# Emilianogith/MPC-for-dynamic-locomotion-in-the-MIT-cheetah-3

Hardware: AMD Instinct MI355X
Metric: QP solves/sec (horizon=10, 4-contact Lite3) at batch=4096 (higher is better)
Workload: dtype f32 tiles + f64 residuals

## Files before the change

mpc-for-dynamic-locomotion-in-the-mit-cheetah-3_amd/csrc/mpcqp_kernels.hip:

```cpp

#include "mpcqp_wrench.h"
#include "mpcqp_stage.h"
#include "mpcqp_elementwise.h"
#include "mpcqp_model.h"
#include "mpcqp_joints.h"

#include <cstdio>
#include <cstdlib>
#include <cstring>
#include <new>
#include <type_traits>

#ifndef MPCQP_DIAG_LDSPAD
#define MPCQP_DIAG_LDSPAD 0
#endif

struct mpcqp_engine {
  MpcQpConfig cfg;
  DevCfg dev;
  DevCfg* dcfg = nullptr;
  hipEvent_t ev0 = nullptr, ev1 = nullptr;
  int* order_mem = nullptr;
  int order_phase = 0;
  int order_cap = 0;
// ... 276 lines not shown
}

static bool invert_small(int n, const double* A, double* Ai) {
  double* M = new (std::nothrow) double[2 * n * n];
  if (!M) return false;
  for (int i = 0; i < n; ++i)
    for (int j = 0; j < n; ++j) { M[i * 2 * n + j] = A[i * n + j]; M[i * 2 * n + n + j] = i == j ? 1.0 : 0.0; }
  bool ok = true;
  for (int k = 0; k < n && ok; ++k) {
    int piv = k;
    for (int i = k + 1; i < n; ++i) if (fabs(M[i * 2 * n + k]) > fabs(M[piv * 2 * n + k])) piv = i;
    if (!(fabs(M[piv * 2 * n + k]) > 0)) { ok = false; break; }
    if (piv != k) for (int j = 0; j < 2 * n; ++j) { const double t = M[k * 2 * n + j]; M[k * 2 * n + j] = M[piv * 2 * n + j]; M[piv * 2 * n + j] = t; }
    const double p = 1.0 / M[k * 2 * n + k];
    for (int j = 0; j < 2 * n; ++j) M[k * 2 * n + j] *= p;
    for (int i = 0; i < n; ++i) {
      if (i == k) continue;
      const double f = M[i * 2 * n + k];
      if (f != 0) for (int j = 0; j < 2 * n; ++j) M[i * 2 * n + j] -= f * M[k * 2 * n + j];
    }
  }
  if (ok) for (int i = 0; i < n; ++i) for (int j = 0; j < n; ++j) Ai[i * n + j] = M[i * 2 * n + n + j];
  delete[] M;
  return ok;
}

template <int N>
static void lane_order_kinv(const double* Ki, double* lane) {
  constexpr int G = WG<N>::G, NQ = WG<N>::NQ;
  auto S0 = [&](int R, int C) -> double {
    if (R >= NQ || C >= NQ) return R == C ? 1.0 : 0.0;
    return R % 6 == C % 6 ? Ki[((R % 6) * N + R / 6) * N + C / 6] : 0.0;
  };
  for (int t = 0; t < G * G; ++t) {
    const int gr = t / G, gc = t % G, k = ((gr - gc) % 3 + 3) % 3;
    for (int r = 0; r < 8; ++r) {
      const int c0 = (r + 2 * k) % 6;
      lane[16 * t + r] = S0(8 * gr + r, 8 * gc + c0);
      lane[16 * t + 8 + r] = c0 < 2 ? S0(8 * gr + r, 8 * gc + c0 + 6) : 0.0;
    }
  }
}

template <int N>
static int build_wrench_tables(mpcqp_engine* e) {
  const MpcQpConfig& c = e->cfg;
  double* tab = new (std::nothrow) double[2 * N * N];
  double* K = new (std::nothrow) double[6 * N * N];
  double* Ki = new (std::nothrow) double[6 * N * N];
  float* Ki32 = new (std::nothrow) float[6 * N * N];
  constexpr int NLANE = 16 * WG<N>::NT;
  double* Kl = new (std::nothrow) double[NLANE];
  float* Kl32 = new (std::nothrow) float[NLANE];
  int rc = tab && K && Ki && Ki32 && Kl && Kl32 ? MPCQP_OK : MPCQP_ENOMEM;
  if (rc == MPCQP_OK) {
    const double dl = c.delta, th = e->dev.theta;
    for (int a = 0; a < N; ++a)
      for (int bq = 0; bq < N; ++bq) {
        const int mx = a > bq ? a : bq;
        tab[a * N + bq] = dl * dl * (double)(N - mx);
        double sacc = 0;
        for (int k = mx + 1; k <= N; ++k) sacc += ((double)(k - 1 - a) + th) * ((double)(k - 1 - bq) + th);
        tab[N * N + a * N + bq] = dl * dl * dl * dl * sacc;
      }
  }
  for (int q = 0; q < 6 && rc == MPCQP_OK; ++q) {
    for (int i = 0; i < N * N; ++i) K[q * N * N + i] = 2.0 * (c.w[q] * tab[N * N + i] + c.w[6 + q] * tab[i]);
    if (!invert_small(N, K + q * N * N, Ki + q * N * N)) rc = MPCQP_EINVAL;
  }
  if (rc == MPCQP_OK) {
    for (int i = 0; i < 6 * N * N; ++i) Ki32[i] = (float)Ki[i];
    lane_order_kinv<N>(Ki, Kl);
    for (int i = 0; i < NLANE; ++i) Kl32[i] = (float)Kl[i];
    hipError_t he = hipMalloc((void**)&e->wr_K, sizeof(double) * 6 * N * N);
    if (he == hipSuccess) he = hipMemcpy(e->wr_K, K, sizeof(double) * 6 * N * N, hipMemcpyHostToDevice);
    if (he == hipSuccess) he = hipMalloc((void**)&e->wr_kinv32, sizeof(float) * 6 * N * N);
    if (he == hipSuccess) he = hipMemcpy(e->wr_kinv32, Ki32, sizeof(float) * 6 * N * N, hipMemcpyHostToDevice);
    if (he == hipSuccess) he = hipMalloc((void**)&e->wr_kinv64, sizeof(double) * 6 * N * N);
    if (he == hipSuccess) he = hipMemcpy(e->wr_kinv64, Ki, sizeof(double) * 6 * N * N, hipMemcpyHostToDevice);
    if (he == hipSuccess) he = hipMalloc((void**)&e->wr_klane32, sizeof(float) * NLANE);
    if (he == hipSuccess) he = hipMemcpy(e->wr_klane32, Kl32, sizeof(float) * NLANE, hipMemcpyHostToDevice);
    if (he == hipSuccess) he = hipMalloc((void**)&e->wr_klane64, sizeof(double) * NLANE);
    if (he == hipSuccess) he = hipMemcpy(e->wr_klane64, Kl, sizeof(double) * NLANE, hipMemcpyHostToDevice);
    if (he != hipSuccess) { (void)hipGetLastError(); rc = MPCQP_ENOMEM; }
  }
  delete[] tab; delete[] K; delete[] Ki; delete[] Ki32; delete[] Kl; delete[] Kl32;
  return rc;
}

static void free_engine(mpcqp_engine* h) {
  if (h->dcfg) (void)hipFree(h->dcfg);
  if (h->order_mem) (void)hipFree(h->order_mem);
  if (h->dual_mem) (void)hipFree(h->dual_mem);
  if (h->model_mem) (void)hipFree(h->model_mem);
  if (h->gait_mem) (void)hipFree(h->gait_mem);
  if (h->roll_mem) (void)hipFree(h->roll_mem);
  if (h->plan_ws) (void)hipFree(h->plan_ws);
  if (h->wr_K) (void)hipFree(h->wr_K);
  if (h->wr_kinv32) (void)hipFree(h->wr_kinv32);
  if (h->wr_kinv64) (void)hipFree(h->wr_kinv64);
  if (h->wr_klane32) (void)hipFree(h->wr_klane32);
  if (h->wr_klane64) (void)hipFree(h->wr_klane64);
  if (h->stage_ws) (void)hipFree(h->stage_ws);
  if (h->ev0) (void)hipEventDestroy(h->ev0);
  if (h->ev1) (void)hipEventDestroy(h->ev1);
  delete h;
}

extern "C" {

uint32_t mpcqp_version(void) { return MPCQP_VERSION; }

int mpcqp_default_config(MpcQpConfig* c) {
  if (!c) return MPCQP_EINVAL;
  memset(c, 0, sizeof(*c));
  c->size = (uint32_t)sizeof(*c);
  c->N = 10;
  c->delta = 0.03;
  c->m = 8.885;
  c->Ibody_inv[0] = 1.0 / 0.24; c->Ibody_inv[1] = 1.0; c->Ibody_inv[2] = 1.0;
  const double w[13] = {1e4, 2.7e4, 1e4, 2.7e5, 2.7e5, 2.7e5, 1e4, 1e4, 1e4, 1.6e4, 1.6e4, 1.6e4, 0.0};
  memcpy(c->w, w, sizeof(w));
  c->alpha = 1e-2;
  c->f_min = 3.0; c->f_max = 100.0;
  c->disc = MPCQP_DISC_EULER;
  c->dtype = MPCQP_DTYPE_F32;
  c->precision = MPCQP_PREC_MIXED;
  c->flags = MPCQP_FLAG_POLISH;
  c->rho = 1.0; c->sigma = 1e-6; c->relax = 1.6;
  c->max_iter = 400; c->check_every = 100;
  c->eps_abs = 1e-5; c->eps_rel = 1e-6;
  c->polish_max = 4;
  c->device = 0;
  return MPCQP_OK;
}

int mpcqp_create(const MpcQpConfig* cfg, mpcqp_handle* out) {
  if (!cfg || !out || cfg->size != sizeof(MpcQpConfig)) return MPCQP_EINVAL;
  *out = nullptr;
// ... 623 lines not shown
```

mpc-for-dynamic-locomotion-in-the-mit-cheetah-3_amd/csrc/mpcqp_leg.h:

```cpp
#pragma once
#include "mpcqp_common.h"
#include "mpcqp_legmap.h"

namespace {

__device__ __forceinline__ int opaque(int v) { asm volatile("" : "+v"(v)); return v; }
__device__ __forceinline__ double opaque_zero_f64() {
  unsigned lo, hi;
  asm volatile("v_mov_b32 %0, 0\n\tv_mov_b32 %1, 0" : "=v"(lo), "=v"(hi));
  return __builtin_bit_cast(double, ((unsigned long long)hi << 32) | lo);
}
template <typename T> __device__ __forceinline__ T opaque_zero() {
  if constexpr (sizeof(T) == 8) return (T)opaque_zero_f64();
  else { float z; asm volatile("v_mov_b32 %0, 0" : "=v"(z)); return (T)z; }
}
__device__ __forceinline__ float ufloat(float v) { return __builtin_bit_cast(float, __builtin_amdgcn_readfirstlane(__builtin_bit_cast(int, v))); }

template <int NW>
__device__ __forceinline__ void wsync() {
  if constexpr (NW == 1) {
    __builtin_amdgcn_fence(__ATOMIC_RELEASE, "wavefront");
    __builtin_amdgcn_wave_barrier();
    __builtin_amdgcn_fence(__ATOMIC_ACQUIRE, "wavefront");
  } else {
    __syncthreads();
  }
}

template <int Q, int NW>
__device__ __forceinline__ void wmax(float (&v)[Q], float* red, int tid) {
  if constexpr (NW == 1) {
#pragma unroll
    for (int q = 0; q < Q; ++q) v[q] = wave_max(v[q]);
  } else {
    block_max<Q, NW>(v, red, tid);
  }
}

template <int Q, int NW>
__device__ __forceinline__ void wsum(float (&v)[Q], float* red, int tid) {
  if constexpr (NW == 1) {
#pragma unroll
    for (int q = 0; q < Q; ++q) v[q] = wave_sum(v[q]);
  } else {
    block_sum<Q, NW>(v, red, tid);
  }
}

template <typename T> __device__ __forceinline__ T quad_sum(T v) { v += dpp_mov<0xB1>(v); v += dpp_mov<0x4E>(v); return v; }

template <typename T>
__device__ __forceinline__ T rs8(const T (&v)[8], int gc) {
  const bool hi = (gc & 4) != 0, b1 = (gc & 2) != 0, b0 = (gc & 1) != 0;
  T t[4];
#pragma unroll
  for (int m = 0; m < 4; ++m) { const T keep = hi ? v[4 + m] : v[m], send = hi ? v[m] : v[4 + m]; t[m] = keep + dpp_mov<0x141>(send); }
  T s2[2];
#pragma unroll
  for (int m = 0; m < 2; ++m) { const T keep = b1 ? t[2 + m] : t[m], send = b1 ? t[m] : t[2 + m]; s2[m] = keep + dpp_mov<0x4E>(send); }
  const T keep = b0 ? s2[1] : s2[0], send = b0 ? s2[0] : s2[1];
  return keep + dpp_mov<0xB1>(send);
}

__device__ __forceinline__ float w_rcp(float x) { return __builtin_amdgcn_rcpf(x); }
__device__ __forceinline__ double w_rcp(double x) {
  double r = __builtin_amdgcn_rcp(x);
  r = fma(fma(-x, r, 1.0), r, r);
  r = fma(fma(-x, r, 1.0), r, r);
  return r;
}

template <typename TM> __device__ __forceinline__ void ld8(const TM* p, TM (&o)[8]);
template <> __device__ __forceinline__ void ld8<float>(const float* p, float (&o)[8]) {
  const float4 a = reinterpret_cast<const float4*>(p)[0], b = reinterpret_cast<const float4*>(p)[1];
  o[0] = a.x; o[1] = a.y; o[2] = a.z; o[3] = a.w; o[4] = b.x; o[5] = b.y; o[6] = b.z; o[7] = b.w;
}
template <> __device__ __forceinline__ void ld8<double>(const double* p, double (&o)[8]) {
#pragma unroll
  for (int h = 0; h < 4; ++h) { const double2 a = reinterpret_cast<const double2*>(p)[h]; o[2 * h] = a.x; o[2 * h + 1] = a.y; }
}
template <typename TM> __device__ __forceinline__ void st8(TM* p, const TM (&o)[8]);
template <> __device__ __forceinline__ void st8<float>(float* p, const float (&o)[8]) {
  reinterpret_cast<float4*>(p)[0] = make_float4(o[0], o[1], o[2], o[3]);
  reinterpret_cast<float4*>(p)[1] = make_float4(o[4], o[5], o[6], o[7]);
}
template <> __device__ __forceinline__ void st8<double>(double* p, const double (&o)[8]) {
#pragma unroll
  for (int h = 0; h < 4; ++h) reinterpret_cast<double2*>(p)[h] = make_double2(o[2 * h], o[2 * h + 1]);
}


template <typename TM>
struct LegAdmm {
  TM u[3], z[5], yh[5], g[3];
  TM lo0, hi0, loA, hiB;
  TM mu;
};

struct ActSet {
  int zs, xs, ys;
  bool ez, ex, ey;
  __device__ __forceinline__ ActSet(int code, bool stance) {
    zs = (code & 3) - 1; xs = ((code >> 2) & 3) - 1; ys = ((code >> 4) & 3) - 1;
    ez = stance && zs == 0; ex = stance && xs == 0; ey = stance && ys == 0;
  }
};

#ifndef MPCQP_AA_M
#define MPCQP_AA_M 3
#endif
constexpr int AA_M = MPCQP_AA_M;
constexpr int AA_NS = 2 * AA_M;
constexpr int AA_NC = AA_M * (AA_M - 1) / 2;
// ... 172 lines not shown
```

mpc-for-dynamic-locomotion-in-the-mit-cheetah-3_amd/csrc/mpcqp_wrench.h:

```cpp
#pragma once
#include "mpcqp_leg.h"

namespace {

template <int N_>
struct WG {
  static constexpr int N = N_, NL = 4 * N, n = 12 * N, NQ = 6 * N;
  static constexpr int G = N <= 10 ? 8 : 16;
  static constexpr int NT = G * G, NW = NT / 64;
  static constexpr int DP = 8 * G;
  static constexpr int NB = (NQ + 7) / 8;
  static_assert(NQ <= DP, "horizon too long for the lane grid");
};

struct WrTabs {
  const double* K;
  const float* kinv32;
  const double* kinv64;
  const float* klane32;
  const double* klane64;
};

template <typename TV, int N>
struct SmemW {
  using Geo = WG<N>;
  TV x0[13];
  TV mu, cy, sy;
  TV rzw0[3];
  TV wP[6], wQ[6];
  TV delta, theta, alpha, inv_m, fmin, fmax;
  TV alpha_target, alpha_ok;
  TV Bl[Geo::NL * 9];
  TV cm[Geo::NL];
  TV gam[Geo::NQ];
  TV gl[Geo::n];
  TV uv[Geo::n];
  TV ww[Geo::NQ], kap[Geo::NQ];
  union {
    struct { TV pu[Geo::n], py[Geo::NL * 5]; };
    struct { TV rr[Geo::n]; TV xd[(N + 1) * 13]; };
  };
  union {
    struct { TV ua[Geo::n], za[Geo::NL * 5], ya[Geo::NL * 5]; };
    struct { TV e0P[Geo::NQ], e0Q[Geo::NQ]; };
  };
  alignas(16) double E[N * 36];
  alignas(16) double piv[2 * Geo::DP];
  alignas(16) double bv[Geo::DP], cv[Geo::DP];
  float red[Geo::NW * 4];
  float aared[Geo::NW * 12];
  float aah[N > 10 ? 45 * Geo::NL : 1];
  float kkt[4];
  float resid[4];
// ... 94 lines not shown

__device__ __forceinline__ void ld4(const float* p, float (&o)[4]) {
  const f2 a = reinterpret_cast<const f2*>(p)[0], b = reinterpret_cast<const f2*>(p)[1];
  o[0] = a.x; o[1] = a.y; o[2] = b.x; o[3] = b.y;
}
__device__ __forceinline__ void ld4(const double* p, double (&o)[4]) {
  const double2 a = reinterpret_cast<const double2*>(p)[0], b = reinterpret_cast<const double2*>(p)[1];
  o[0] = a.x; o[1] = a.y; o[2] = b.x; o[3] = b.y;
}

__device__ __forceinline__ float wmasked(float x, int m) { return __builtin_bit_cast(float, __builtin_bit_cast(int, x) & m); }
__device__ __forceinline__ double wmasked(double x, int m) { return __builtin_bit_cast(double, __builtin_bit_cast(long long, x) & (long long)m); }

template <typename TM, int N, bool VM>
__device__ __forceinline__ void w_tile_init(WTile<TM>& t, const WKq<TM>& kq, const TM* __restrict__ E, int gr, int gc) {
  constexpr int NQ = WG<N>::NQ, G = WG<N>::G;
  asm volatile("" : "+v"(gr), "+v"(gc));
  const unsigned cls = (unsigned)(gr - gc + 3 * G) % 3u;
  const bool kc[3] = {cls == 0u, cls == 1u, cls == 2u};
#pragma unroll
  for (int r = 0; r < 8; ++r) {
    TM kv[8];
#pragma unroll
    for (int c = 0; c < 8; ++c) {
      TM v = (TM)0;
#pragma unroll
      for (int k = 0; k < 3; ++k) {
        const int c0 = (r + 2 * k) % 6;
        if (c == c0) v = kc[k] ? kq.v0[r] : v;
        else if (c == c0 + 6) v = kc[k] ? kq.v1[r] : v;
      }
      kv[c] = v;
    }
    const int R = 8 * gr + r, jR = (R * 43) >> 8;
    const int h = R < NQ ? 3 * jR - 4 * gc : 64;
    const int base = 6 * R - 2 * h;
    const unsigned bits = ((7u << min((unsigned)(h + 2), 31u)) >> 2) & 15u;
#pragma unroll
    for (int hq = 0; hq < 2; ++hq) {
      const bool in0 = (unsigned)(2 * hq - h) < 3u, in1 = (unsigned)(2 * hq + 1 - h) < 3u;
      TM e[4];
      if constexpr (VM) ld4(E + ((bits & (3u << (2 * hq))) ? base + 4 * hq : 0), e);
      else ld4(E + ((in0 || in1) ? base + 4 * hq : 0), e);
#pragma unroll
      for (int i = 0; i < 4; ++i) {
        const int c = 4 * hq + i;
        if constexpr (VM) tset(t, r, c, kv[c] + wmasked(e[i], __builtin_amdgcn_sbfe((int)bits, 2 * hq + (i >> 1), 1)));
        else tset(t, r, c, kv[c] + ((i < 2 ? in0 : in1) ? e[i] : (TM)0));
      }
    }
  }
}

template <typename TM, int N>
__device__ __forceinline__ void w_sweep(WTile<TM>& t, TM* __restrict__ piv, int gr, int gc) {
  constexpr int NW = WG<N>::NW, DP = WG<N>::DP, G = WG<N>::G;
  int step = 0;
  for (int og = 0; og < G; ++og) {
#pragma unroll
    for (int rr = 0; rr < 8; ++rr) {
      if (8 * og + rr >= WG<N>::NQ) break;
      TM* vb = piv + (NW > 1 ? (step & 1) * DP : 0);
      if (gr == og) {
        TM row[8];
#pragma unroll
        for (int j = 0; j < 8; ++j) row[j] = tget(t, rr, j);
        st8<TM>(vb + 8 * gc, row);
      }
      wsync<NW>();
      const TM p = w_rcp(vb[8 * og + rr]);
      TM vc[8], vr[8];
      ld8<TM>(vb + 8 * gc, vc);
      ld8<TM>(vb + 8 * gr, vr);
      const bool prow = gr == og, pcol = gc == og;
      TM m[8];
#pragma unroll
      for (int i = 0; i < 8; ++i) { vr[i] *= p; m[i] = vr[i]; }
      m[rr] = prow ? (TM)1 - p : vr[rr];
      rank1(t, m, vc);
#pragma unroll
      for (int i = 0; i < 8; ++i) {
        const TM v = (i == rr && prow) ? -p : vr[i];
        tset(t, i, rr, pcol ? v : tget(t, i, rr));
      }
      if constexpr (NW == 1) wsync<1>();
      tpin(t);
      ++step;
    }
  }
}

template <typename TM, int N, bool NEGATE = true>
__device__ __forceinline__ void w_matvec(const WTile<TM>& t, const TM* __restrict__ bv, TM* __restrict__ cv, int gr, int gc) {
  constexpr int G = WG<N>::G;
  TM x[8], acc[8];
  ld8<TM>(bv + 8 * gc, x);
  tilemv(t, x, acc);
  if constexpr (G == 16) {
#pragma unroll
    for (int i = 0; i < 8; ++i) acc[i] += dpp_mov<0x140>(acc[i]);
  }
  const TM sum = rs8<TM>(acc, gc & 7), tot = NEGATE ? -sum : sum;
  if (gc < 8) cv[8 * gr + gc] = tot;
}

template <int N, bool MIXED> constexpr bool W_LEGMAP = N == 10 && MIXED;
template <int N, bool MIXED> constexpr bool W_MED3 = N == 10 && MIXED;

template <typename TM, int N, typename LS>
__device__ __forceinline__ void w_build_E(const LS& L, TM* __restrict__ E, int tid) {
  constexpr int NL = WG<N>::NL, NW = WG<N>::NW;
  TM e[21];
  int k = 0;
  if constexpr (LS::dense) {
#pragma unroll
    for (int q = 0; q < 6; ++q) {
#pragma unroll
      for (int p = q; p < 6; ++p) {
        TM a = L.dinv[0] * L.A[0][q] * L.A[0][p];
        a = fma(L.dinv[1] * L.A[1][q], L.A[1][p], a);
        a = fma(L.dinv[2] * L.A[2][q], L.A[2][p], a);
        e[k++] = quad_sum(a);
      }
    }
  } else {
    L.gram(e, [](TM a) { return quad_sum(a); });
  }
  if (tid < NL && (tid & 3) == 0) {
    TM* Ej = E + 36 * (tid >> 2);
    k = 0;
#pragma unroll
    for (int q = 0; q < 6; ++q) {
#pragma unroll
      for (int p = q; p < 6; ++p) { Ej[6 * q + p] = e[k]; Ej[6 * p + q] = e[k]; ++k; }
    }
  }
  wsync<NW>();
}

template <typename TM, int N, bool QUAD_PIN = false, typename LS>
__device__ __forceinline__ void w_solve(const WTile<TM>& t, const LS& L, const TM (&rhs)[3], TM (&x)[3], TM* __restrict__ bv,
                                        TM* __restrict__ cv, int tid, int gr, int gc) {
  constexpr int NL = WG<N>::NL, NW = WG<N>::NW;
  TM a[3];
#pragma unroll
  for (int c = 0; c < 3; ++c) a[c] = L.dinv[c] * rhs[c];
  TM b[6];
  static_assert(!QUAD_PIN || (sizeof(TM) == 4 && !LS::dense), "the pinned form is written for fp32 on the structured maps");
  if constexpr (LS::dense) {
#pragma unroll
    for (int q = 0; q < 6; ++q) b[q] = quad_sum(fma(L.A[2][q], a[2], fma(L.A[1][q], a[1], L.A[0][q] * a[0])));
  } else if constexpr (!QUAD_PIN) {
    L.wrench(a, b, [](TM v) { return quad_sum(v); });
  } else {
    L.wrench(a, b, [](TM v) { return v; });
    typedef float v2f __attribute__((ext_vector_type(2)));
    v2f p01 = {b[0], b[1]}, p34 = {b[3], b[4]};
    asm volatile("" : "+v"(p01), "+v"(p34));
    b[0] = p01.x; b[1] = p01.y; b[3] = p34.x; b[4] = p34.y;
    asm volatile("" : "+v"(b[2]), "+v"(b[5]));
#pragma unroll
    for (int q = 0; q < 6; ++q) b[q] = quad_sum(b[q]);
  }
  {
    const int l = min(tid & 3, 2);
    TM v0 = l == 0 ? b[0] : (l == 1 ? b[2] : b[4]), v1 = l == 0 ? b[1] : (l == 1 ? b[3] : b[5]);
    if constexpr (QUAD_PIN) { asm volatile("" : "+v"(v0)); asm volatile("" : "+v"(v1)); }
    if (tid < NL) { TM* d = bv + 6 * (tid >> 2) + 2 * l; d[0] = v0; d[1] = v1; }
  }
  wsync<NW>();
  w_matvec<TM, N, !QUAD_PIN>(t, bv, cv, gr, gc);
  wsync<NW>();
  const TM* cj = cv + 6 * (min(tid, NL - 1) >> 2);
  TM c6[6];
#pragma unroll
  for (int q = 0; q < 6; ++q) c6[q] = QUAD_PIN ? -cj[q] : cj[q];
  if constexpr (LS::dense) {
#pragma unroll
    for (int c = 0; c < 3; ++c) {
      TM s = L.A[c][0] * c6[0];
#pragma unroll
      for (int q = 1; q < 6; ++q) s = fma(L.A[c][q], c6[q], s);
      x[c] = a[c] - L.dinv[c] * s;
    }
  } else {
    L.back(c6, [&](const int c, const TM sc) { x[c] = a[c] - L.dinv[c] * sc; });
  }
}

template <typename TV, typename TIO, int N>
__device__ __forceinline__ int w_load(SmemW<TV, N>& s, const FastIn<TIO>& in, size_t b, int tid) {
  constexpr int NT = WG<N>::NT, n = WG<N>::n, NL = WG<N>::NL, NX = (N + 1) * 13;
  constexpr int RX = (NX + NT - 1) / NT, RR = (n + NT - 1) / NT, RC = (NL + NT - 1) / NT;
  TIO vx[RX], vr[RR], v0 = 0, vm = 0;
  uint8_t vc[RC];
  const TIO* xp = in.xdes + b * (size_t)NX;
  const TIO* rp = in.r + b * (size_t)n;
  const uint8_t* cp = in.contact + b * (size_t)NL;
#pragma unroll
  for (int q = 0; q < RX; ++q) { const int i = tid + q * NT; vx[q] = i < NX ? xp[i] : (TIO)0; }
#pragma unroll
  for (int q = 0; q < RR; ++q) { const int i = tid + q * NT; vr[q] = i < n ? rp[i] : (TIO)0; }
#pragma unroll
  for (int q = 0; q < RC; ++q) { const int i = tid + q * NT; vc[q] = i < NL ? cp[i] : (uint8_t)0; }
  if (tid < 13) v0 = in.x0[b * 13 + tid];
  if (tid == 0) vm = in.mu[b];
  int bad = 0;
#pragma unroll
  for (int q = 0; q < RX; ++q) { const int i = tid + q * NT; if (i < NX) { s.xd[i] = (TV)vx[q]; bad |= !isfinite(vx[q]); } }
#pragma unroll
  for (int q = 0; q < RR; ++q) { const int i = tid + q * NT; if (i < n) { s.rr[i] = (TV)vr[q]; bad |= !isfinite(vr[q]); } }
#pragma unroll
  for (int q = 0; q < RC; ++q) { const int i = tid + q * NT; if (i < NL) s.ct[i] = vc[q] ? 1 : 0; }
  if (tid < 13) { s.x0[tid] = (TV)v0; bad |= !isfinite(v0); }
  if (tid == 0) { s.mu = (TV)vm; bad |= !isfinite(vm); }
  return bad;
}

template <typename TV, int N>
__device__ __forceinline__ void w_grad(SmemW<TV, N>& s, const double* __restrict__ Ktab, int tid, TV (&gr)[3]) {
  constexpr int NL = WG<N>::NL, NQ = WG<N>::NQ, NW = WG<N>::NW, NT = WG<N>::NT;
  static_assert(NQ <= NT, "one wrench component per lane");
  const int L = min(tid, NL - 1);
  const int e = min(tid, NQ - 1), ej = e / 6, eq = e - 6 * ej;
// ... 271 lines not shown
  TV u[3], z[5], y[5], g[3];
#pragma unroll
  for (int a = 0; a < 3; ++a) { u[a] = s.ua[3 * L + a]; g[a] = s.gl[3 * L + a]; }
#pragma unroll
  for (int i = 0; i < 5; ++i) { z[i] = s.za[5 * L + i]; y[i] = s.ya[5 * L + i]; }
  return w_ratio<TV, N>(s, tabs, u, z, y, g, s.mu, tid < NL, tid);
}

constexpr double ALPHA_FLOOR = 3e-6;
constexpr int POLISH_CHEAP_LEGS = 3;
constexpr int POLISH_CHEAP_STEPS = 3;
constexpr int POLISH_PATIENCE = 1;

template <typename TV, typename TM, int N, typename LS>
__device__ __forceinline__ void w_admm_sys(const SmemW<TV, N>& s, const DevCfg& cfg, int L, float rho, LS& Ls) {
  const bool stance = s.ct[L] != 0;
  if constexpr (LS::dense) {
#pragma unroll
    for (int c = 0; c < 3; ++c) {
#pragma unroll
      for (int i = 0; i < 3; ++i) Ls.A[c][i] = (TM)s.Bl[9 * L + 3 * i + c];
#pragma unroll
      for (int a = 0; a < 3; ++a) Ls.A[c][3 + a] = a == c ? (TM)s.cm[L] : (TM)0;
    }
  } else {
#pragma unroll
    for (int c = 0; c < 3; ++c) {
#pragma unroll
      for (int i = 0; i < 3; ++i) Ls.B[c][i] = (TM)s.Bl[9 * L + 3 * i + c];
    }
    Ls.cm = (TM)s.cm[L];
  }
  TM sigma = (TM)cfg.sigma;
  if constexpr (sizeof(TM) == 4) sigma = ufloat(sigma);
  const TM r = (TM)rho, m = (TM)s.mu, a2 = (TM)((TV)2 * s.alpha);
  if constexpr (!LS::dense) {
    const TM base = a2 + sigma;
    Ls.dinv[0] = Ls.dinv[1] = stance ? (TM)1 / (base + (r + r)) : (TM)0;
    Ls.dinv[2] = stance ? (TM)1 / fma(r, fma((TM)4 * m, m, (TM)1), base) : (TM)0;
  } else {
    Ls.dinv[0] = Ls.dinv[1] = stance ? (TM)1 / (a2 + sigma + (TM)2 * r) : (TM)0;
    Ls.dinv[2] = stance ? (TM)1 / (a2 + sigma + r * fma((TM)4 * m, m, (TM)1)) : (TM)0;
  }
}

template <typename TV, typename TM, int N, bool REFINE = false>
__device__ __forceinline__ void w_admm(SmemW<TV, N>& s, const DevCfg& cfg, const WrTabs& tabs, const int adapt,
                                       const int kfirst, const int tid0) {
  constexpr int NL = WG<N>::NL, NW = WG<N>::NW, G = WG<N>::G;
  constexpr bool AA_CARRY = NW == 1 && !REFINE && sizeof(TM) == 4;
  constexpr bool LM = W_LEGMAP<N, sizeof(TM) == 4>;
  static_assert(!LM || (NW == 1 && sizeof(TM) == 4), "w_solve's pinned quad sums are written for one wave and fp32");
  constexpr bool MED3 = W_MED3<N, sizeof(TM) == 4>;
  using TS = std::conditional_t<(N > 10), double, TM>;
  TM* const E = reinterpret_cast<TM*>(s.E);
  TM* const piv = reinterpret_cast<TM*>(s.piv);
  TM* const bv = reinterpret_cast<TM*>(s.bv);
  TM* const cv = reinterpret_cast<TM*>(s.cv);
  float rho = s.rho;
  int K = kfirst > 0 ? min(kfirst, cfg.check_every) : cfg.check_every;
  K = max(1, min(K, cfg.max_iter - __builtin_amdgcn_readfirstlane(s.iters)));
  const int seg_len = (!REFINE && sizeof(TM) == 4 && cfg.accel_p > 0 && cfg.accel_restart > 0) ? cfg.accel_restart : (1 << 30);
  const bool check = adapt && cfg.early_check;
  int it = 0, seg_end = min(K, (adapt && ADAPT_AT < K) ? ADAPT_AT : seg_len);
  int hard = 0;
  float ratio = 0.f;
  STAMP_INIT
  for (;;) {
    WKq<TS> kq;
    {
      const int tid = fresh_tid<NW>(tid0), L = min(tid, NL - 1);
      w_kq_load<TS>(kq, w_klane<TS>(tabs), tid);
      typename LegMapPick<LM, LegMapAdmm<TS>, TS>::type Ls;
      w_admm_sys<TV, TS, N>(s, cfg, L, rho, Ls);
      w_build_E<TS, N>(Ls, reinterpret_cast<TS*>(s.E), tid);
    }
    STAMP(1);
    WTile<TM> tile;
    {
      const int tid = fresh_tid<NW>(tid0), gr = tid / G, gc = tid % G;
      if constexpr (sizeof(TS) == sizeof(TM)) {
        w_tile_init<TM, N, sizeof(TM) == 4>(tile, kq, E, gr, gc);
        STAMP(2);
        w_sweep<TM, N>(tile, piv, gr, gc);
      } else {
        WTile<TS> t64;
        w_tile_init<TS, N, sizeof(TM) == 4>(t64, kq, reinterpret_cast<const TS*>(s.E), gr, gc);
        STAMP(2);
        w_sweep<TS, N>(t64, reinterpret_cast<TS*>(s.piv), gr, gc);
#pragma unroll
        for (int i = 0; i < 8; ++i) {
#pragma unroll
          for (int j = 0; j < 4; ++j) tile.v[i][j] = mk2((float)t64.v[i][2 * j], (float)t64.v[i][2 * j + 1]);
        }
      }
    }
    STAMP(3);
    {
      const int tid = fresh_tid<NW>(tid0), L = min(tid, NL - 1), gr = tid / G, gc = tid % G;
      const bool leg = tid < NL, stance = s.ct[L] != 0;
      const TM sigma = (TM)cfg.sigma, relax = (TM)cfg.relax, om = (TM)1 - relax, BIG = (TM)1e30, r = (TM)rho;
      if (tid >= WG<N>::NQ && tid < WG<N>::DP) bv[tid] = (TM)0;
      typename LegMapPick<LM, LegMapAdmm<TM>, TM>::type Ls;
      w_admm_sys<TV, TM, N>(s, cfg, L, rho, Ls);
      LegAdmm<TM> A;
      A.mu = (TM)s.mu;
#pragma unroll
      for (int a = 0; a < 3; ++a) { A.u[a] = (TM)s.ua[3 * L + a]; A.g[a] = (TM)s.gl[3 * L + a]; }
#pragma unroll
      for (int i = 0; i < 5; ++i) { A.z[i] = (TM)s.za[5 * L + i]; A.yh[i] = (TM)(s.ya[5 * L + i] / (TV)rho); }
      A.lo0 = stance ? (TM)s.fmin : (TM)0; A.hi0 = stance ? (TM)s.fmax : (TM)0;
      A.loA = stance ? -BIG : (TM)0; A.hiB = stance ? BIG : (TM)0;
      bool rebuild = false;
      constexpr bool AA_ON = !REFINE && sizeof(TM) == 4, AA_LDS = N > 10;
      const int aa_p = AA_ON ? __builtin_amdgcn_readfirstlane(cfg.accel_p) : 0;
      LegAA aa;
      TM aa_xb[5], aa_fp[5];
      auto aa_park = [&]() {
        if constexpr (AA_LDS) {
          if (leg) {
            float* h = s.aah + L;
#pragma unroll
            for (int k = 0; k < 5; ++k) {
              h[NL * k] = (float)aa_xb[k]; h[NL * (5 + k)] = (float)aa_fp[k]; h[NL * (10 + k)] = aa.rp[k];
#pragma unroll
              for (int j = 0; j < AA_M; ++j) { h[NL * (15 + 5 * j + k)] = aa.dX[j][k]; h[NL * (15 + 5 * AA_M + 5 * j + k)] = aa.dF[j][k]; }
            }
          }
        }
      };
      auto aa_fetch = [&]() {
        if constexpr (AA_LDS) {
          const float* h = s.aah + L;
#pragma unroll
          for (int k = 0; k < 5; ++k) {
            aa_xb[k] = (TM)h[NL * k]; aa_fp[k] = (TM)h[NL * (5 + k)]; aa.rp[k] = h[NL * (10 + k)];
#pragma unroll
// ... 141 lines not shown
    if (y0 + (u2 - fmaxv) > 0) zs = 1;
    else if (y0 + (u2 - fminv) < 0) zs = -1;
    const bool hx = y1 + g1 > 0, lx = y2 + g2 < 0;
    if (hx && lx) xs = (g1 > -g2) ? 1 : -1; else if (hx) xs = 1; else if (lx) xs = -1;
    const bool hy = y3 + g3_ > 0, ly = y4 + g4 < 0;
    if (hy && ly) ys = (g3_ > -g4) ? 1 : -1; else if (hy) ys = 1; else if (ly) ys = -1;
  }
  return (zs + 1) | ((xs + 1) << 2) | ((ys + 1) << 4);
}

template <typename TV, int N>
__device__ __forceinline__ unsigned w_aset_hash(SmemW<TV, N>& s, const int tid) {
  constexpr int NL = WG<N>::NL, NW = WG<N>::NW;
  if (tid == 0) s.ahash = 0u;
  wsync<NW>();
  if (tid < NL) atomicAdd(&s.ahash, ((unsigned)s.aset[tid] + 1u) * (2654435761u * (unsigned)(2 * tid + 1)));
  wsync<NW>();
  const unsigned h = (unsigned)__builtin_amdgcn_readfirstlane((int)s.ahash);
  wsync<NW>();
  return h;
}

#ifndef MPCQP_W_INCR_LEGS
#define MPCQP_W_INCR_LEGS 8
#endif
#ifndef MPCQP_W_INCR_STEPS
#define MPCQP_W_INCR_STEPS 12
#endif

template <typename TV, typename TP, int N, bool VM, bool LM>
__device__ __forceinline__ int w_polish_round(SmemW<TV, N>& s, const WrTabs& tabs, const int tid0,
                                              const int budget, const bool last, const int trace_tag, const int incr_legs,
                                              const int patience, const int cheap_steps, const int cheap_legs, const int last_patience) {
  constexpr int NL = WG<N>::NL, NW = WG<N>::NW, G = WG<N>::G;
  using PMap = typename LegMapPick<LM, LegMapPolish<TP>, TP>::type;
  constexpr int STG = 2 * 21 + 1;
  static_assert(STG * MPCQP_W_INCR_LEGS <= N * 36, "the staging records share the bytes of E");
  TP* const E = reinterpret_cast<TP*>(s.E);
  TP* const piv = reinterpret_cast<TP*>(s.piv);
  TP* const bv = reinterpret_cast<TP*>(s.bv);
  TP* const cv = reinterpret_cast<TP*>(s.cv);
  STAMP_INIT
  {
    const int tid = fresh_tid<NW>(tid0), L = min(tid, NL - 1);
    const int code = w_polish_rule<TV, N>(s, L, s.ct[L] != 0);
    if (tid < NL) s.aset[L] = (uint8_t)code;
    wsync<NW>();
    const unsigned h0 = w_aset_hash<TV, N>(s, tid);
    if (tid == 0) s.ahist[0] = h0;
  }
  int ok = 0, ps = 0, nstall = 0, cheap_used = 0;
  float vprev = INFINITY, vprev2 = INFINITY;
  bool done = false;
  while (!done) {
    WKq<TP> kq;
    {
      const int tid = fresh_tid<NW>(tid0), L = min(tid, NL - 1);
      w_kq_load<TP>(kq, w_klane<TP>(tabs), tid);
      PMap Ls;
      w_polish_sys<TV, TP, N>(s, L, ActSet(s.aset[L], s.ct[L] != 0), Ls);
      w_build_E<TP, N>(Ls, E, tid);
    }
    STAMP(9);
    WTile<TP> tile;
    {
      const int tid = fresh_tid<NW>(tid0), gr = tid / G, gc = tid % G;
      w_tile_init<TP, N, VM>(tile, kq, E, gr, gc);
      STAMP(10);
      w_sweep<TP, N>(tile, piv, gr, gc);
    }
    STAMP(11);
    int in_row = 0;
    for (;;) {
      int step_ok_i;
      {
      const int tid = fresh_tid<NW>(tid0), L = min(tid, NL - 1), gr = tid / G, gc = tid % G;
      const bool leg = tid < NL, stance = s.ct[L] != 0;
      if (tid >= WG<N>::NQ && tid < WG<N>::DP) bv[tid] = opaque_zero<TP>();
      const ActSet as(s.aset[L], stance);
      const int zs = as.zs, xs = as.xs, ys = as.ys;
      const bool ez = as.ez, ex = as.ex, ey = as.ey;
      TV txs, tys;
      TV v3[3];
      {
        const TV muv = s.mu;
        txs = (TV)xs * muv; tys = (TV)ys * muv;
        const TV F = zs > 0 ? (TV)s.fmax : (TV)s.fmin;
        v3[0] = ex ? s.pu[3 * L] : (TV)0; v3[1] = ey ? s.pu[3 * L + 1] : (TV)0;
        v3[2] = ez ? s.pu[3 * L + 2] : ((stance && zs != 0) ? F : (TV)0);
      }
      TV uc[3], gr3[3] = {0, 0, 0};
      auto expand = [&]() {
        uc[2] = v3[2];
        uc[0] = ex ? v3[0] : txs * v3[2];
        uc[1] = ey ? v3[1] : tys * v3[2];
      };
      float stat = INFINITY, prev = INFINITY;
      for (int rf = 0;; ++rf) {
        expand();
        if (leg) {
    #pragma unroll
          for (int c = 0; c < 3; ++c) s.uv[3 * L + c] = uc[c];
        }
        wsync<NW>();
        w_grad<TV, N>(s, tabs.K, tid, gr3);
        TV rg[3] = {ex ? gr3[0] : (TV)0, ey ? gr3[1] : (TV)0, ez ? gr3[2] + txs * gr3[0] + tys * gr3[1] : (TV)0};
        float q[2] = {leg ? fmaxf(fmaxf(fabsf((float)rg[0]), fabsf((float)rg[1])), fabsf((float)rg[2])) : 0.f,
                      leg ? fmaxf(fmaxf(fabsf((float)uc[0]), fabsf((float)uc[1])), fabsf((float)uc[2])) : 0.f};
        if (!isfinite(q[0])) q[0] = INFINITY;
        wmax<2, NW>(q, s.red, tid);
        prev = stat; stat = ufloat(q[0]);
        const float gmaxl = s.gmax;
        const float tol_stat = (sizeof(TV) == 8) ? (1e-6f + 1e-9f * gmaxl) : (3e-7f * fmaxf(gmaxl, 1.f));
        const float tol = fminf(tol_stat, 0.25f * ((sizeof(TV) == 8) ? 2.f * (float)s.alpha : 1e30f) * 2e-5f * fmaxf(1.f, q[1]));
        if (stat <= tol || rf >= 4 || (rf > 0 && !(stat < 0.5f * prev))) break;
        const TP rhs[3] = {(TP)(-rg[0]), (TP)(-rg[1]), (TP)(-rg[2])};
        TP dx[3];
        {
          PMap Ls;
          w_polish_sys<TV, TP, N>(s, L, as, Ls);
// ... 366 lines not shown
```

Baseline: 12.20 million.

## Precompute per-lane row offset tables for tile init, add banked DPP reduce and packed multiplies

Adds a host-built per-lane record that packs the lane-ordered K-inverse values together with row words encoding E offsets and pair masks. The tile-init step then uses those words to do direct quad loads from E with masks, instead of computing indices per row. Separately, the matvec reduction gains a banked DPP first stage written in inline asm, and the elimination sweep uses packed fp32 two-wide multiplies for the pivot-row scaling. All three apply only to the N=10 fp32 path and add table memory plus hand-written asm that depends on the lane layout.

```diff
diff --git a/mpc-for-dynamic-locomotion-in-the-mit-cheetah-3_amd/csrc/mpcqp_kernels.hip b/mpc-for-dynamic-locomotion-in-the-mit-cheetah-3_amd/csrc/mpcqp_kernels.hip
--- a/mpc-for-dynamic-locomotion-in-the-mit-cheetah-3_amd/csrc/mpcqp_kernels.hip
+++ b/mpc-for-dynamic-locomotion-in-the-mit-cheetah-3_amd/csrc/mpcqp_kernels.hip
@@ -352,7 +352,12 @@
   constexpr int NLANE = 16 * WG<N>::NT;
   double* Kl = new (std::nothrow) double[NLANE];
   float* Kl32 = new (std::nothrow) float[NLANE];
-  int rc = tab && K && Ki && Ki32 && Kl && Kl32 ? MPCQP_OK : MPCQP_ENOMEM;
+  constexpr int NREC = N == 10 ? WG<N>::NT : 0;
+  constexpr size_t L32 = sizeof(float) * NLANE + NREC * mpcqp_rowtab::record_bytes<float>();
+  constexpr size_t L64 = sizeof(double) * NLANE + NREC * mpcqp_rowtab::record_bytes<double>();
+  unsigned* rows = new (std::nothrow) unsigned[mpcqp_rowtab::ROW_WORDS * WG<N>::NT];
+  unsigned char* img = new (std::nothrow) unsigned char[L32 + L64];
+  int rc = tab && K && Ki && Ki32 && Kl && Kl32 && rows && img ? MPCQP_OK : MPCQP_ENOMEM;
   if (rc == MPCQP_OK) {
     const double dl = c.delta, th = e->dev.theta;
     for (int a = 0; a < N; ++a)
@@ -368,6 +373,7 @@
     for (int i = 0; i < N * N; ++i) K[q * N * N + i] = 2.0 * (c.w[q] * tab[N * N + i] + c.w[6 + q] * tab[i]);
     if (!invert_small(N, K + q * N * N, Ki + q * N * N)) rc = MPCQP_EINVAL;
   }
+  if (rc == MPCQP_OK && NREC > 0 && !mpcqp_rowtab::lane_order_rows(N, WG<N>::G, rows)) rc = MPCQP_EINVAL;
   if (rc == MPCQP_OK) {
     for (int i = 0; i < 6 * N * N; ++i) Ki32[i] = (float)Ki[i];
     lane_order_kinv<N>(Ki, Kl);
@@ -378,13 +384,19 @@
     if (he == hipSuccess) he = hipMemcpy(e->wr_kinv32, Ki32, sizeof(float) * 6 * N * N, hipMemcpyHostToDevice);
     if (he == hipSuccess) he = hipMalloc((void**)&e->wr_kinv64, sizeof(double) * 6 * N * N);
     if (he == hipSuccess) he = hipMemcpy(e->wr_kinv64, Ki, sizeof(double) * 6 * N * N, hipMemcpyHostToDevice);
-    if (he == hipSuccess) he = hipMalloc((void**)&e->wr_klane32, sizeof(float) * NLANE);
-    if (he == hipSuccess) he = hipMemcpy(e->wr_klane32, Kl32, sizeof(float) * NLANE, hipMemcpyHostToDevice);
-    if (he == hipSuccess) he = hipMalloc((void**)&e->wr_klane64, sizeof(double) * NLANE);
-    if (he == hipSuccess) he = hipMemcpy(e->wr_klane64, Kl, sizeof(double) * NLANE, hipMemcpyHostToDevice);
+    memcpy(img, Kl32, sizeof(float) * NLANE);
+    memcpy(img + L32, Kl, sizeof(double) * NLANE);
+    if (NREC > 0) {
+      mpcqp_rowtab::pack_records<float>(NREC, Kl32, rows, img + sizeof(float) * NLANE);
+      mpcqp_rowtab::pack_records<double>(NREC, Kl, rows, img + L32 + sizeof(double) * NLANE);
+    }
+    if (he == hipSuccess) he = hipMalloc((void**)&e->wr_klane32, L32);
+    if (he == hipSuccess) he = hipMemcpy(e->wr_klane32, img, L32, hipMemcpyHostToDevice);
+    if (he == hipSuccess) he = hipMalloc((void**)&e->wr_klane64, L64);
+    if (he == hipSuccess) he = hipMemcpy(e->wr_klane64, img + L32, L64, hipMemcpyHostToDevice);
     if (he != hipSuccess) { (void)hipGetLastError(); rc = MPCQP_ENOMEM; }
   }
-  delete[] tab; delete[] K; delete[] Ki; delete[] Ki32; delete[] Kl; delete[] Kl32;
+  delete[] tab; delete[] K; delete[] Ki; delete[] Ki32; delete[] Kl; delete[] Kl32; delete[] rows; delete[] img;
   return rc;
 }
 
diff --git a/mpc-for-dynamic-locomotion-in-the-mit-cheetah-3_amd/csrc/mpcqp_leg.h b/mpc-for-dynamic-locomotion-in-the-mit-cheetah-3_amd/csrc/mpcqp_leg.h
--- a/mpc-for-dynamic-locomotion-in-the-mit-cheetah-3_amd/csrc/mpcqp_leg.h
+++ b/mpc-for-dynamic-locomotion-in-the-mit-cheetah-3_amd/csrc/mpcqp_leg.h
@@ -59,6 +59,27 @@
 #pragma unroll
   for (int m = 0; m < 2; ++m) { const T keep = b1 ? t[2 + m] : t[m], send = b1 ? t[m] : t[2 + m]; s2[m] = keep + dpp_mov<0x4E>(send); }
   const T keep = b0 ? s2[1] : s2[0], send = b0 ? s2[0] : s2[1];
+  return keep + dpp_mov<0xB1>(send);
+}
+
+__device__ __forceinline__ float rs8_banked(const float (&v)[8], int gc) {
+  const bool b1 = (gc & 2) != 0, b0 = (gc & 1) != 0;
+  float t[4];
+  asm("s_nop 1\n\t"
+      "v_add_f32_dpp %0, %4, %4 row_half_mirror row_mask:0xf bank_mask:0x5\n\t"
+      "v_add_f32_dpp %1, %5, %5 row_half_mirror row_mask:0xf bank_mask:0x5\n\t"
+      "v_add_f32_dpp %2, %6, %6 row_half_mirror row_mask:0xf bank_mask:0x5\n\t"
+      "v_add_f32_dpp %3, %7, %7 row_half_mirror row_mask:0xf bank_mask:0x5\n\t"
+      "v_add_f32_dpp %0, %8, %8 row_half_mirror row_mask:0xf bank_mask:0xa\n\t"
+      "v_add_f32_dpp %1, %9, %9 row_half_mirror row_mask:0xf bank_mask:0xa\n\t"
+      "v_add_f32_dpp %2, %10, %10 row_half_mirror row_mask:0xf bank_mask:0xa\n\t"
+      "v_add_f32_dpp %3, %11, %11 row_half_mirror row_mask:0xf bank_mask:0xa"
+      : "=&v"(t[0]), "=&v"(t[1]), "=&v"(t[2]), "=&v"(t[3])
+      : "v"(v[0]), "v"(v[1]), "v"(v[2]), "v"(v[3]), "v"(v[4]), "v"(v[5]), "v"(v[6]), "v"(v[7]));
+  float s2[2];
+#pragma unroll
+  for (int m = 0; m < 2; ++m) { const float keep = b1 ? t[2 + m] : t[m], send = b1 ? t[m] : t[2 + m]; s2[m] = keep + dpp_mov<0x4E>(send); }
+  const float keep = b0 ? s2[1] : s2[0], send = b0 ? s2[0] : s2[1];
   return keep + dpp_mov<0xB1>(send);
 }
 
diff --git a/mpc-for-dynamic-locomotion-in-the-mit-cheetah-3_amd/csrc/mpcqp_rowtab.h b/mpc-for-dynamic-locomotion-in-the-mit-cheetah-3_amd/csrc/mpcqp_rowtab.h
--- /dev/null
+++ b/mpc-for-dynamic-locomotion-in-the-mit-cheetah-3_amd/csrc/mpcqp_rowtab.h
@@ -0,0 +1,55 @@
+#pragma once
+#include <cstring>
+
+namespace mpcqp_rowtab {
+
+constexpr int PAIR_BIT = 12;
+constexpr int QUAD_STEP = 16;
+
+constexpr int row_h(int N, int gr, int gc, int r) {
+  const int R = 8 * gr + r;
+  return R < 6 * N ? 3 * (R / 6) - 4 * gc : 64;
+}
+constexpr unsigned row_pairs(int N, int gr, int gc, int r) {
+  const int h = row_h(N, gr, gc, r);
+  unsigned bits = 0;
+  for (int p = 0; p < 4; ++p) bits |= (unsigned)(h <= p && p <= h + 2) << p;
+  return bits;
+}
+constexpr int row_quad(int N, int gr, int gc, int r, int hq) {
+  const int R = 8 * gr + r, base = 6 * R - 2 * row_h(N, gr, gc, r);
+  return (row_pairs(N, gr, gc, r) & (3u << (2 * hq))) ? base + 4 * hq : 0;
+}
+constexpr unsigned row_word(int N, int gr, int gc, int r) {
+  return 8u * (unsigned)row_quad(N, gr, gc, r, 0) | row_pairs(N, gr, gc, r) << PAIR_BIT | 8u * (unsigned)row_quad(N, gr, gc, r, 1) << QUAD_STEP;
+}
+
+inline bool lane_order_rows(int N, int G, unsigned* tab) {
+  bool ok = true;
+  for (int t = 0; t < G * G; ++t) {
+    for (int r = 0; r < 8; ++r) {
+      for (int hq = 0; hq < 2; ++hq) {
+        const int o = row_quad(N, t / G, t % G, r, hq);
+        ok = ok && o >= 0 && o + 4 <= 36 * N && 8 * o < (1 << PAIR_BIT) && o % 2 == 0;
+      }
+      tab[8 * t + r] = row_word(N, t / G, t % G, r);
+    }
+  }
+  return ok;
+}
+
+constexpr int LANE_VALUES = 16, ROW_WORDS = 8;
+template <typename T> constexpr int record_words_at() { return LANE_VALUES * (int)sizeof(T); }
+template <typename T> constexpr int record_bytes() { return record_words_at<T>() + ROW_WORDS * (int)sizeof(unsigned); }
+static_assert(record_bytes<float>() % 16 == 0 && record_bytes<double>() % 16 == 0, "b128 loads of a record");
+
+template <typename T>
+inline void pack_records(int nlane, const T* values, const unsigned* words, unsigned char* out) {
+  for (int t = 0; t < nlane; ++t) {
+    unsigned char* rec = out + (std::size_t)t * record_bytes<T>();
+    std::memcpy(rec, values + LANE_VALUES * t, LANE_VALUES * sizeof(T));
+    std::memcpy(rec + record_words_at<T>(), words + ROW_WORDS * t, ROW_WORDS * sizeof(unsigned));
+  }
+}
+
+}
diff --git a/mpc-for-dynamic-locomotion-in-the-mit-cheetah-3_amd/csrc/mpcqp_wrench.h b/mpc-for-dynamic-locomotion-in-the-mit-cheetah-3_amd/csrc/mpcqp_wrench.h
--- a/mpc-for-dynamic-locomotion-in-the-mit-cheetah-3_amd/csrc/mpcqp_wrench.h
+++ b/mpc-for-dynamic-locomotion-in-the-mit-cheetah-3_amd/csrc/mpcqp_wrench.h
@@ -1,4 +1,5 @@
 #pragma once
+#include "mpcqp_rowtab.h"
 #include "mpcqp_leg.h"
 
 namespace {
@@ -199,7 +200,56 @@
   }
 }
 
+struct WRows { unsigned w[8]; };
+
 template <typename TM, int N>
+__device__ __forceinline__ void w_kq_rows_load(WKq<TM>& k, WRows& rw, const TM* __restrict__ klane, int tid) {
+  using namespace mpcqp_rowtab;
+  static_assert(LANE_VALUES == 16 && ROW_WORDS == 8, "v0[8] | v1[8] and WRows::w[8]");
+  const char* rec = reinterpret_cast<const char*>(klane + LANE_VALUES * WG<N>::NT) + record_bytes<TM>() * tid;
+  ld8<TM>(reinterpret_cast<const TM*>(rec), k.v0);
+  ld8<TM>(reinterpret_cast<const TM*>(rec) + 8, k.v1);
+  const uint4 a = reinterpret_cast<const uint4*>(rec + record_words_at<TM>())[0], b = reinterpret_cast<const uint4*>(rec + record_words_at<TM>())[1];
+  rw.w[0] = a.x; rw.w[1] = a.y; rw.w[2] = a.z; rw.w[3] = a.w; rw.w[4] = b.x; rw.w[5] = b.y; rw.w[6] = b.z; rw.w[7] = b.w;
+}
+
+template <typename TM, int N>
+__device__ __forceinline__ void w_tile_init_rows(WTile<TM>& t, const WKq<TM>& kq, const WRows& rw, const TM* __restrict__ E, int gr, int gc) {
+  constexpr int G = WG<N>::G;
+  using namespace mpcqp_rowtab;
+  asm volatile("" : "+v"(gr), "+v"(gc));
+  const unsigned cls = (unsigned)(gr - gc + 3 * G) % 3u;
+  const bool kc[3] = {cls == 0u, cls == 1u, cls == 2u};
+#pragma unroll
+  for (int r = 0; r < 8; ++r) {
+    TM kv[8];
+#pragma unroll
+    for (int c = 0; c < 8; ++c) {
+      TM v = (TM)0;
+#pragma unroll
+      for (int k = 0; k < 3; ++k) {
+        const int c0 = (r + 2 * k) % 6;
+        if (c == c0) v = kc[k] ? kq.v0[r] : v;
+        else if (c == c0 + 6) v = kc[k] ? kq.v1[r] : v;
+      }
+      kv[c] = v;
+    }
+    const unsigned w = rw.w[r];
+#pragma unroll
+    for (int hq = 0; hq < 2; ++hq) {
+      const unsigned off = sizeof(TM) == 4 ? __builtin_amdgcn_ubfe(w, QUAD_STEP * hq + 1, PAIR_BIT - 1) : __builtin_amdgcn_ubfe(w, QUAD_STEP * hq, PAIR_BIT);
+      TM e[4];
+      ld4(reinterpret_cast<const TM*>(reinterpret_cast<const char*>(E) + off), e);
+#pragma unroll
+      for (int i = 0; i < 4; ++i) {
+        const int c = 4 * hq + i;
+        tset(t, r, c, kv[c] + wmasked(e[i], __builtin_amdgcn_sbfe((int)w, PAIR_BIT + 2 * hq + (i >> 1), 1)));
+      }
+    }
+  }
+}
+
+template <typename TM, int N, bool PKMUL = false>
 __device__ __forceinline__ void w_sweep(WTile<TM>& t, TM* __restrict__ piv, int gr, int gc) {
   constexpr int NW = WG<N>::NW, DP = WG<N>::DP, G = WG<N>::G;
   int step = 0;
@@ -222,7 +272,15 @@
       const bool prow = gr == og, pcol = gc == og;
       TM m[8];
 #pragma unroll
-      for (int i = 0; i < 8; ++i) { vr[i] *= p; m[i] = vr[i]; }
+      for (int i = 0; i < 8; ++i) {
+        if constexpr (PKMUL) {
+          static_assert(sizeof(TM) == 4, "packed multiplies are fp32");
+          if (i % 2 == 0) { const f2 s = mk2(vr[i], vr[i + 1]) * splat2(p); vr[i] = s.x; vr[i + 1] = s.y; }
+        } else {
+          vr[i] *= p;
+        }
+        m[i] = vr[i];
+      }
       m[rr] = prow ? (TM)1 - p : vr[rr];
       rank1(t, m, vc);
 #pragma unroll
@@ -237,7 +295,7 @@
   }
 }
 
-template <typename TM, int N, bool NEGATE = true>
+template <typename TM, int N, bool NEGATE = true, bool BANKED = false>
 __device__ __forceinline__ void w_matvec(const WTile<TM>& t, const TM* __restrict__ bv, TM* __restrict__ cv, int gr, int gc) {
   constexpr int G = WG<N>::G;
   TM x[8], acc[8];
@@ -247,12 +305,22 @@
 #pragma unroll
     for (int i = 0; i < 8; ++i) acc[i] += dpp_mov<0x140>(acc[i]);
   }
-  const TM sum = rs8<TM>(acc, gc & 7), tot = NEGATE ? -sum : sum;
+  TM sum;
+  if constexpr (BANKED) {
+    static_assert(G == 8 && sizeof(TM) == 4, "rs8_banked: lane = 8 gr + gc of one wave, fp32");
+    sum = rs8_banked(acc, gc & 7);
+  } else {
+    sum = rs8<TM>(acc, gc & 7);
+  }
+  const TM tot = NEGATE ? -sum : sum;
   if (gc < 8) cv[8 * gr + gc] = tot;
 }
 
 template <int N, bool MIXED> constexpr bool W_LEGMAP = N == 10 && MIXED;
 template <int N, bool MIXED> constexpr bool W_MED3 = N == 10 && MIXED;
+template <int N, bool MIXED> constexpr bool W_TRIM_RS8 = N == 10 && MIXED;
+template <int N, bool MIXED> constexpr bool W_TRIM_PKMUL = N == 10 && MIXED;
+template <int N, bool MIXED> constexpr bool W_TRIM_ROWTAB = N == 10 && MIXED;
 
 template <typename TM, int N, typename LS>
 __device__ __forceinline__ void w_build_E(const LS& L, TM* __restrict__ E, int tid) {
@@ -316,7 +384,7 @@
     if (tid < NL) { TM* d = bv + 6 * (tid >> 2) + 2 * l; d[0] = v0; d[1] = v1; }
   }
   wsync<NW>();
-  w_matvec<TM, N, !QUAD_PIN>(t, bv, cv, gr, gc);
+  w_matvec<TM, N, !QUAD_PIN, QUAD_PIN && W_TRIM_RS8<N, sizeof(TM) == 4>>(t, bv, cv, gr, gc);
   wsync<NW>();
   const TM* cj = cv + 6 * (min(tid, NL - 1) >> 2);
   TM c6[6];
@@ -694,6 +762,7 @@
   constexpr bool LM = W_LEGMAP<N, sizeof(TM) == 4>;
   static_assert(!LM || (NW == 1 && sizeof(TM) == 4), "w_solve's pinned quad sums are written for one wave and fp32");
   constexpr bool MED3 = W_MED3<N, sizeof(TM) == 4>;
+  constexpr bool ROWTAB = W_TRIM_ROWTAB<N, sizeof(TM) == 4>;
   using TS = std::conditional_t<(N > 10), double, TM>;
   TM* const E = reinterpret_cast<TM*>(s.E);
   TM* const piv = reinterpret_cast<TM*>(s.piv);
@@ -710,9 +779,11 @@
   STAMP_INIT
   for (;;) {
     WKq<TS> kq;
+    WRows rw;
     {
       const int tid = fresh_tid<NW>(tid0), L = min(tid, NL - 1);
-      w_kq_load<TS>(kq, w_klane<TS>(tabs), tid);
+      if constexpr (ROWTAB) w_kq_rows_load<TS, N>(kq, rw, w_klane<TS>(tabs), tid);
+      else w_kq_load<TS>(kq, w_klane<TS>(tabs), tid);
       typename LegMapPick<LM, LegMapAdmm<TS>, TS>::type Ls;
       w_admm_sys<TV, TS, N>(s, cfg, L, rho, Ls);
       w_build_E<TS, N>(Ls, reinterpret_cast<TS*>(s.E), tid);
@@ -721,10 +792,15 @@
     WTile<TM> tile;
     {
       const int tid = fresh_tid<NW>(tid0), gr = tid / G, gc = tid % G;
-      if constexpr (sizeof(TS) == sizeof(TM)) {
+      if constexpr (ROWTAB) {
+        static_assert(!ROWTAB || sizeof(TS) == sizeof(TM), "kq and rw were loaded in the sweep's element type: the row table serves a tile that is built and swept in TM");
+        w_tile_init_rows<TM, N>(tile, kq, rw, E, gr, gc);
+        STAMP(2);
+        w_sweep<TM, N, W_TRIM_PKMUL<N, sizeof(TM) == 4>>(tile, piv, gr, gc);
+      } else if constexpr (sizeof(TS) == sizeof(TM)) {
         w_tile_init<TM, N, sizeof(TM) == 4>(tile, kq, E, gr, gc);
         STAMP(2);
-        w_sweep<TM, N>(tile, piv, gr, gc);
+        w_sweep<TM, N, W_TRIM_PKMUL<N, sizeof(TM) == 4>>(tile, piv, gr, gc);
       } else {
         WTile<TS> t64;
         w_tile_init<TS, N, sizeof(TM) == 4>(t64, kq, reinterpret_cast<const TS*>(s.E), gr, gc);
@@ -972,11 +1048,14 @@
   int ok = 0, ps = 0, nstall = 0, cheap_used = 0;
   float vprev = INFINITY, vprev2 = INFINITY;
   bool done = false;
+  constexpr bool ROWTAB = W_TRIM_ROWTAB<N, VM>;
   while (!done) {
     WKq<TP> kq;
+    WRows rw;
     {
       const int tid = fresh_tid<NW>(tid0), L = min(tid, NL - 1);
-      w_kq_load<TP>(kq, w_klane<TP>(tabs), tid);
+      if constexpr (ROWTAB) w_kq_rows_load<TP, N>(kq, rw, w_klane<TP>(tabs), tid);
+      else w_kq_load<TP>(kq, w_klane<TP>(tabs), tid);
       PMap Ls;
       w_polish_sys<TV, TP, N>(s, L, ActSet(s.aset[L], s.ct[L] != 0), Ls);
       w_build_E<TP, N>(Ls, E, tid);
@@ -985,7 +1064,8 @@
     WTile<TP> tile;
     {
       const int tid = fresh_tid<NW>(tid0), gr = tid / G, gc = tid % G;
-      w_tile_init<TP, N, VM>(tile, kq, E, gr, gc);
+      if constexpr (ROWTAB) w_tile_init_rows<TP, N>(tile, kq, rw, E, gr, gc);
+      else w_tile_init<TP, N, VM>(tile, kq, E, gr, gc);
       STAMP(10);
       w_sweep<TP, N>(tile, piv, gr, gc);
     }
```

Measured after the change: 12.54 million, median of 6. 2.7% higher.
